# Virtana/accurate-aprilgroup-tracking

Measured on AMD Instinct MI355X. Metric: frames/sec (LK+PnP) on 1280x720 dodeca stream, higher is better.
Workload: dtype u8/i64 (LK), f64 (PnP); 1 GPU; c2: 1 x 1280x720 stream(s) per GPU, 12 tags/48 corners, 3-level LK 21x21, iterative PnP with motion-model guess; streams_per_gpu=1, frames_resident=HBM ring 368 slots (323 MiB), parallelism=stream-per-GPU x1, RCCL all_gather of poses once per block

## Files before the change

### accurate_aprilgroup_tracking_amd/csrc/agt_device.h

```cpp
#pragma once
#include <hip/hip_runtime.h>
#include <stdint.h>
#include <float.h>

#define AGT_WAVE 64

__device__ __forceinline__ int agt_reflect101(int p, int len)
{
    if ((unsigned)p < (unsigned)len) return p;
    if (len == 1) return 0;
    do {
        p = p < 0 ? -p : 2 * (len - 1) - p;
    } while ((unsigned)p >= (unsigned)len);
    return p;
}

template <int CTRL>
__device__ __forceinline__ int agt_dpp_i32(int v)
{
    return __builtin_amdgcn_update_dpp(0, v, CTRL, 0xf, 0xf, true);
}

__device__ __forceinline__ long long agt_dpp_add_i64_step(long long v, int lo, int hi)
{
// ... 26 lines not shown
}

__device__ __forceinline__ int agt_uniform(int v) { return __builtin_amdgcn_readfirstlane(v); }
__device__ __forceinline__ float agt_uniform(float v)
{
    return __int_as_float(__builtin_amdgcn_readfirstlane(__float_as_int(v)));
}

#pragma clang fp contract(fast)

__device__ __forceinline__ double agt_rcp(double x)
{
    double r = __builtin_amdgcn_rcp(x);
    double e = __builtin_fma(-x, r, 1.0);
    r = __builtin_fma(r, e, r);
    e = __builtin_fma(-x, r, 1.0);
    return __builtin_fma(r, e, r);
}
__device__ __forceinline__ double agt_rcp1(double x)
{
    const double r = __builtin_amdgcn_rcp(x);
    return __builtin_fma(r, __builtin_fma(-x, r, 1.0), r);
}
__device__ __forceinline__ double agt_sqrtp(double x)
{
    if (x == 0.0) return 0.0;
    const double y = __builtin_amdgcn_rsq(x);
    double g = x * y, h = 0.5 * y;
    double r = __builtin_fma(-h, g, 0.5);
    g = __builtin_fma(g, r, g); h = __builtin_fma(h, r, h);
    const double d = __builtin_fma(-g, g, x);
    return __builtin_fma(d, h, g);
}


__device__ __forceinline__ void agt_sincos(double x, double& s, double& c)
{
    if (!(x < 1048576.0)) { sincos(x, &s, &c); return; }
    const double k = rint(x * 6.36619772367581382433e-01);
    double r = fma(-k, 1.57079632673412561417e+00, x);
    r = fma(-k, 6.07710050650619224932e-11, r);
    const double z = r * r;
    const double sp = fma(z, fma(z, fma(z, fma(z, fma(z, 1.58969099521155010221e-10, -2.50507602534068634195e-08), 2.75573137070700676789e-06),
                                       -1.98412698298579493134e-04), 8.33333333332248946124e-03), -1.66666666666666324348e-01);
    const double cp = fma(z, fma(z, fma(z, fma(z, fma(z, -1.13596475577881948265e-11, 2.08757232129817482790e-09), -2.75573143513906633035e-07),
                                       2.48015872894767294178e-05), -1.38888888888741095749e-03), 4.16666666666666019037e-02);
    const double sr = fma(r * z, sp, r);
    const double cr = fma(z * z, cp, fma(z, -0.5, 1.0));
    const int q = (int)k & 3;
    const double ss = (q & 1) ? cr : sr, cc = (q & 1) ? sr : cr;
    s = (q & 2) ? -ss : ss;
    c = ((q + 1) & 2) ? -cc : cc;
}

template <bool JAC>
__device__ __forceinline__ void agt_rodrigues(const double r_in[3], double R[9], double G[9])
{
    double rx = r_in[0], ry = r_in[1], rz = r_in[2];
    const double t2 = rx * rx + ry * ry + rz * rz;
    const double theta = agt_sqrtp(t2);
    const bool tiny = theta < DBL_EPSILON;
    double s, c;
    agt_sincos(theta, s, c);
    const double c1 = 1.0 - c, itheta = agt_rcp(tiny ? 1.0 : theta);
    if (JAC) {
        double a, bq;
        if (theta < 1e-2) {
            a = 0.5 - t2 * (1.0 / 24.0 - t2 * (1.0 / 720.0 - t2 * (1.0 / 40320.0)));
            bq = 1.0 / 6.0 - t2 * (1.0 / 120.0 - t2 * (1.0 / 5040.0 - t2 * (1.0 / 362880.0)));
        } else {
            const double it2 = itheta * itheta;
            a = c1 * it2;
            bq = (theta - s) * it2 * itheta;
        }
        const double d = 1.0 - bq * t2;
        const double g[9] = { d + bq * rx * rx, bq * rx * ry - a * rz, bq * rx * rz + a * ry,
                              bq * rx * ry + a * rz, d + bq * ry * ry, bq * ry * rz - a * rx,
                              bq * rx * rz - a * ry, bq * ry * rz + a * rx, d + bq * rz * rz };
#pragma unroll
        for (int i = 0; i < 9; i++) G[i] = tiny ? ((i % 4 == 0) ? 1.0 : 0.0) : g[i];
    }
    rx *= itheta; ry *= itheta; rz *= itheta;
    const double rrt[9] = { rx * rx, rx * ry, rx * rz, rx * ry, ry * ry, ry * rz, rx * rz, ry * rz, rz * rz };
    const double r_x[9] = { 0, -rz, ry, rz, 0, -rx, -ry, rx, 0 };
#pragma unroll
    for (int k = 0; k < 9; k++) {
        const double v = c * ((k % 4 == 0) ? 1.0 : 0.0) + c1 * rrt[k] + s * r_x[k];
        R[k] = tiny ? ((k % 4 == 0) ? 1.0 : 0.0) : v;
    }
}

struct AgtCamera {
    double fx, fy, cx, cy;
    double k[12];
    const double* tilt;
};

__device__ __forceinline__ void agt_tilt_apply(const double* M, double x, double y, double& xo, double& yo, double* d)
{
    double v[3];
#pragma unroll
    for (int r = 0; r < 3; r++) { double a = 0.0; a += M[r * 3] * x; a += M[r * 3 + 1] * y; a += M[r * 3 + 2] * 1.0; v[r] = a; }
    const double ip = v[2] != 0.0 ? 1.0 / v[2] : 1.0;
    xo = ip * v[0]; yo = ip * v[1];
    if (d) {
        const double ip2 = ip * ip;
#pragma unroll
        for (int r = 0; r < 2; r++)
#pragma unroll
            for (int c = 0; c < 2; c++) d[r * 2 + c] = (M[r * 3 + c] * v[2] - M[6 + c] * v[r]) * ip2;
    }
}

template <bool JAC, bool DIST = true>
__device__ __forceinline__ void agt_project(const AgtCamera& cam, const double R[9], const double G[9],
                                            const double t[3], double X, double Y, double Z,
                                            double& u, double& v, double jr[6], double jt[6])
{
    const double* k = cam.k;
    const double wx = R[0] * X + R[1] * Y + R[2] * Z;
    const double wy = R[3] * X + R[4] * Y + R[5] * Z;
    const double wz = R[6] * X + R[7] * Y + R[8] * Z;
    double x = wx + t[0];
    double y = wy + t[1];
    double z = wz + t[2];
    z = z != 0.0 ? agt_rcp(z) : 1.0;
    x *= z; y *= z;
    if (!DIST) {
        u = x * cam.fx + cam.cx;
        v = y * cam.fy + cam.cy;
        if (JAC) {
            jt[0] = cam.fx * z; jt[1] = 0.0; jt[2] = cam.fx * (-x * z);
            jt[3] = 0.0; jt[4] = cam.fy * z; jt[5] = cam.fy * (-y * z);
#pragma unroll
            for (int j = 0; j < 3; j++) {
                const double gx = G[j], gy = G[3 + j], gz = G[6 + j];
                const double dx0 = gy * wz - gz * wy;
                const double dy0 = gz * wx - gx * wz;
                const double dz0 = gx * wy - gy * wx;
                jr[j] = cam.fx * (z * (dx0 - x * dz0));
                jr[3 + j] = cam.fy * (z * (dy0 - y * dz0));
            }
// ... 227 lines not shown
```

### accurate_aprilgroup_tracking_amd/csrc/agt_lk_chain_body.h

```cpp
#pragma once
#include "agt_lk_body.h"

#ifdef AGT_STEP_STAMPS
__device__ unsigned long long agt_chain_stamps[4 * 16];
__device__ unsigned agt_chain_counts[8];
#define CCOUNT(i, n) do { if (threadIdx.x == 0) atomicAdd(&agt_chain_counts[i], (unsigned)(n)); } while (0)
#define CSTAMP(i) do { if (pidx == 0 && threadIdx.x == 0 && k < 4) agt_chain_stamps[k * 16 + (i)] = __builtin_amdgcn_s_memtime(); } while (0)
extern "C" int agt_debug_chain_stamps(unsigned long long* host64)
{
    return (int)hipMemcpyFromSymbol(host64, HIP_SYMBOL(agt_chain_stamps), sizeof(agt_chain_stamps));
}
extern "C" int agt_debug_chain_counts(unsigned* host8)
{
    return (int)hipMemcpyFromSymbol(host8, HIP_SYMBOL(agt_chain_counts), sizeof(agt_chain_counts));
}
#else
#define CSTAMP(i)
#define CCOUNT(i, n)
#endif

#ifdef AGT_CHAIN_REPS
__device__ int agt_chain_reps[8] = { 1, 1, 1, 1, 1, 1, 1, 1 };
extern "C" int agt_debug_chain_reps(const int* host8) { return (int)hipMemcpyToSymbol(HIP_SYMBOL(agt_chain_reps), host8, 32); }
#define CREPS(i) for (int rep_ = 0, n_ = *(volatile int*)&agt_chain_reps[i]; rep_ < n_; rep_++)
// ... 276 lines not shown
            }
            if (sv) *reinterpret_cast<int2*>(sDall + l * (K::SD / 4) + sY * DW + sX) = make_int2(val[0], val[1]);
        }
        lds_barrier();
        CSTAMP(3);

        int Iv[NLEV][C::NPX], Ix[NLEV][C::NPX], Iy[NLEV][C::NPX];
        CREPS(1)
#pragma unroll
        for (int l = 0; l < NLEV; l++) {
            int iw00, iw01, iw10, iw11;
            bilinear_weights(fa[l], fb[l], iw00, iw01, iw10, iw11);
            const uint8_t* s0 = lds + offS[l];
            const int* sD = sDall + l * (K::SD / 4);
            int a0 = 0, a1 = 0, a2 = 0;
#pragma unroll
            for (int q = 0; q < C::NPX; q++) {
                const uint8_t* p = s0 + oW[q];
                const int iv = descale(bil4(p[0], p[1], p[JP], p[JP + 1], iw00, iw01, iw10, iw11), W_BITS - 5);
                const int* d = sD + oD[q];
                const int d00 = d[0], d01 = d[1], d10 = d[DW], d11 = d[DW + 1];
                const int ix = descale(bil4((short)d00, (short)d01, (short)d10, (short)d11, iw00, iw01, iw10, iw11), W_BITS);
                const int iy = descale(bil4(d00 >> 16, d01 >> 16, d10 >> 16, d11 >> 16, iw00, iw01, iw10, iw11), W_BITS);
                Iv[l][q] = pv[q] ? iv : 0; Ix[l][q] = pv[q] ? ix : 0; Iy[l][q] = pv[q] ? iy : 0;
                a0 += __mul24(Ix[l][q], Ix[l][q]); a1 += __mul24(Ix[l][q], Iy[l][q]); a2 += __mul24(Iy[l][q], Iy[l][q]);
            }
            red[(3 * l) * T + tid] = a0; red[(3 * l + 1) * T + tid] = a1; red[(3 * l + 2) * T + tid] = a2;
        }
        lds_barrier();
        CREPS(2)
        for (int l = wave; l < NLEV; l += NW) {
            int s4[3];
#pragma unroll
            for (int i = 0; i < 3; i++) {
                const int* r = red + (3 * l + i) * T + lane;
                s4[i] = r[0] + r[64] + r[128] + r[192];
            }
            int lo[3], hi[3];
            wave_sum2_i32(s4[0] & 0xffff, s4[1] & 0xffff, lo[0], lo[1]);
            wave_sum2_i32(s4[2] & 0xffff, s4[0] >> 16, lo[2], hi[0]);
            wave_sum2_i32(s4[1] >> 16, s4[2] >> 16, hi[1], hi[2]);
            float A[3];
#pragma unroll
            for (int i = 0; i < 3; i++) A[i] = fmaf((float)hi[i], 65536.f, (float)lo[i]) * FLT_SCALE;
            const float D = A[0] * A[2] - A[1] * A[1];
            const float minEig = (A[2] + A[0] - sqrtf((A[0] - A[2]) * (A[0] - A[2]) + 4.f * A[1] * A[1])) / (float)(2 * WIN * WIN);
            const bool ok = ((lvA >> l) & 1) && !((double)minEig < min_eig_threshold || D < FLT_EPSILON);
            if (lane == 0) {
                float* o = lvl + l * 8;
                o[0] = A[0]; o[1] = A[1]; o[2] = A[2]; o[3] = ok ? 1.f / D : 0.f; o[4] = ok ? 1.f : 0.f;
            }
        }
        lds_barrier();
        if (owed && tid == 0) lk_arrive(owed, b);
        owed = nullptr;
        CSTAMP(4);

        int st = 1;
        float outx = 0.f, outy = 0.f;
        bool pre = false;
        uint32_t tn[NLEV][C::JLD];
        int nox[NLEV], noy[NLEV], nmask = 0;
#pragma unroll
        for (int l = 0; l < NLEV; l++) { nox[l] = noy[l] = 0; }
#pragma unroll
        for (int level = NLEV - 1; level >= 0; level--) {
            if (level > maxl) continue;
            const float scale = lk_level_scale(level);
            float nextx, nexty;
            if (level == maxl) { nextx = px * scale; nexty = py * scale; }
            else { nextx = outx * 2.f; nexty = outy * 2.f; }
            outx = nextx; outy = nexty;
            CSTAMP(8 + level * 2);
            if (level == 0 && k + 1 < nf) {
                const LkFrameIo<NLEV> nio = frame(k + 1);
                if (agt_uniform((int)(all_safe && !nio.bad))) {
                    CREPS(4) {
                    nmask = 0;
#pragma unroll
                    for (int l = 0; l < NLEV; l++) {
                        typedef const __attribute__((address_space(1))) uint8_t* G8;
                        typedef const __attribute__((address_space(1))) uint32_t* G32;
                        const float sc = lk_level_scale(l);
                        const int cx = agt_uniform((int)floorf(outx * sc - halfw)), cy = agt_uniform((int)floorf(outy * sc - halfw));
                        const int w = gw[l], h = gh[l];
                        const long pitch = gpitch[l], bstride = gbs[l];
                        const int ox = cx - MARGIN, oy = cy - MARGIN, ax0 = ox & ~3;
                        const bool ok = l <= maxl && ax0 >= 0 && ax0 + 4 * C::JNDW <= w && oy >= 0 && oy + JT <= h;
                        const int lx = ok ? ax0 : 0, ly = ok ? oy : 0;
                        const uint8_t* img = l <= maxl ? nio.imgJ[l] : nio.imgJ[0];
                        const G8 base = (G8)img + (long)b * (l <= maxl ? bstride : 0) + (long)ly * (l <= maxl ? pitch : 0) + lx;
#pragma unroll
                        for (int q = 0; q < C::JLD; q++) tn[l][q] = *(G32)(base + toff[l][q]);
                        nox[l] = ox; noy[l] = oy;
                        nmask |= ok ? 1 << l : 0;
                    }
                    }
                    pre = true;
                }
            }
            if (!((lvA >> level) & 1)) { if (level == 0) st = 0; continue; }
            const float4 lv4 = *reinterpret_cast<const float4*>(lvl + level * 8);
            if (!agt_uniform((int)(lvl[level * 8 + 4] != 0.f))) { if (level == 0) st = 0; continue; }
            AgtLevel LJ;
            LJ.ptr = nullptr; LJ.w = gw[level]; LJ.h = gh[level]; LJ.pitch = gpitch[level]; LJ.bstride = gbs[level];
            const uint8_t* imgJ = io.imgJ[level] + (long)b * LJ.bstride;
            uint8_t* sJ = lds + (cur * NLEV + level) * K::TILE;
            const float a11 = agt_uniform(lv4.x), a12 = agt_uniform(lv4.y), a22 = agt_uniform(lv4.z), D = agt_uniform(lv4.w);
            int iv[C::NPX], ix[C::NPX], iy[C::NPX];
#pragma unroll
            for (int q = 0; q < C::NPX; q++) { iv[q] = Iv[level][q]; ix[q] = Ix[level][q]; iy[q] = Iy[level][q]; }
            int jx0 = jox[level], jy0 = joy[level];

            nextx -= halfw; nexty -= halfw;
            float pdx = 0.f, pdy = 0.f;
            int iw00, iw01, iw10, iw11;
            float bx0, bx1, by0, by1;
            auto set_box = [&]() {
                const int lx = jx0 > -WIN ? jx0 : -WIN, hx = (jx0 + JT - WIN - 1 < LJ.w - 1 ? jx0 + JT - WIN - 1 : LJ.w - 1) + 1;
                const int ly = jy0 > -WIN ? jy0 : -WIN, hy = (jy0 + JT - WIN - 1 < LJ.h - 1 ? jy0 + JT - WIN - 1 : LJ.h - 1) + 1;
                bx0 = (float)lx; bx1 = (float)hx; by0 = (float)ly; by1 = (float)hy;
            };
            set_box();
            int slow = agt_uniform((int)!(nextx >= bx0 && nextx < bx1 && nexty >= by0 && nexty < by1));
            for (int j = 0; j < max_count; j++) {
                const float fx = floorf(nextx), fy = floorf(nexty);
                if (slow) {
                    const int inx = agt_uniform((int)fx), iny = agt_uniform((int)fy);
                    if (inx < -WIN || inx >= LJ.w || iny < -WIN || iny >= LJ.h) {
                        if (level == 0) st = 0;
                        break;
                    }
                    if (inx < jx0 || inx + WIN >= jx0 + JT || iny < jy0 || iny + WIN >= jy0 + JT) {
                        jx0 = inx - MARGIN; jy0 = iny - MARGIN;
                        uint32_t t[C::JLD];
                        block_sync<NW>();
                        tile_load<JT, C::JNDW, T, C::JLD, true>(imgJ, LJ.w, LJ.h, LJ.pitch, jx0, jy0, tid, t);
                        tile_store<JT, C::JNDW, T>(sJ, tid, t);
                        __builtin_amdgcn_s_waitcnt(0x0F70);
                        block_sync<NW>();
                        set_box();
                    }
                }
                const int inx = (int)fx, iny = (int)fy;
                const uint8_t* q0 = sJ + __mul24(iny - jy0, JP) + (inx - jx0) + (jx0 - (jx0 & ~3));
                int tap[C::NPX][4];
#pragma unroll
                for (int q = 0; q < C::NPX; q++) {
                    const uint8_t* c = q0 + oW[q];
                    tap[q][0] = c[0]; tap[q][1] = c[1]; tap[q][2] = c[JP]; tap[q][3] = c[JP + 1];
                }
                __builtin_amdgcn_sched_barrier(0);
                bilinear_weights(nextx - fx, nexty - fy, iw00, iw01, iw10, iw11);
                int bsum[2] = { 0, 0 };
#pragma unroll
                for (int q = 0; q < C::NPX; q++) {
// ... 63 lines not shown
```

### accurate_aprilgroup_tracking_amd/csrc/agt_pnp_body.h

```cpp
#pragma once
#include <type_traits>
#include <cstddef>
#include "agt_device.h"
#include "agt_kernels.h"

#ifdef AGT_PNP_STAMPS
__device__ unsigned long long agt_pnp_stamps[64];
#define PSTAMP(i) do { if (b == 0 && threadIdx.x == 0) agt_pnp_stamps[i] = __builtin_amdgcn_s_memtime(); } while (0)
#define PSTAMPM(i) do { int mk_; asm volatile("s_mov_b32 %0, %1" : "=s"(mk_) : "n"(0xbeef00 + (i))); PSTAMP(i); } while (0)
extern "C" int agt_debug_pnp_stamps(unsigned long long* host64)
{
    return (int)hipMemcpyFromSymbol(host64, HIP_SYMBOL(agt_pnp_stamps), sizeof(agt_pnp_stamps));
}
#else
#define PSTAMP(i)
#define PSTAMPM(i)
#endif

#pragma clang fp contract(fast)

namespace agt_pnp {

constexpr int NACC = 28;
constexpr int SLAB = 65;
constexpr int MAX_PPL = 4;

__device__ __forceinline__ void pnp_sync()
{
    __builtin_amdgcn_fence(__ATOMIC_RELEASE, "wavefront");
    __builtin_amdgcn_wave_barrier();
    __builtin_amdgcn_fence(__ATOMIC_ACQUIRE, "wavefront");
}

struct PnpShared {
    double part[NACC * SLAB];
    double tot[NACC + 4];
    double LL[144];
    double vec[48];
    unsigned long long tab[5 * AGT_MAX_GROUP];
    int seq;
    int late;
    int coop[2];
    AgtTrackState ts;
};

typedef __attribute__((address_space(3))) AgtTrackState AgtTrackStateLds;

template <int K, bool READBACK = true>
__device__ __forceinline__ void wave_reduce_slab(double (&vals)[K], PnpShared& sh, int lane)
{
    static_assert(K <= NACC, "the slab holds NACC rows");
    pnp_sync();
#pragma unroll
    for (int k = 0; k < K; k++) sh.part[k * SLAB + lane] = vals[k];
    pnp_sync();
    const int k = lane & 31, h = lane >> 5;
    double s = 0.0;
    if (k < K) {
        const double* p = &sh.part[k * SLAB + 32 * h];
#pragma unroll 8
        for (int i = 0; i < 32; i++) s += p[i];
    }
    s += __shfl_xor(s, 32);
    if (lane < K) sh.tot[lane] = s;
    pnp_sync();
    if (READBACK) {
#pragma unroll
        for (int i = 0; i < K; i++) vals[i] = sh.tot[i];
    }
}

__device__ __forceinline__ double dswap32(double a, double b, double& b_out)
{
    const auto lo = __builtin_amdgcn_permlane32_swap((unsigned)__double2loint(a), (unsigned)__double2loint(b), false, false);
    const auto hi = __builtin_amdgcn_permlane32_swap((unsigned)__double2hiint(a), (unsigned)__double2hiint(b), false, false);
    b_out = __hiloint2double((int)hi[1], (int)lo[1]);
    return __hiloint2double((int)hi[0], (int)lo[0]);
}
__device__ __forceinline__ double dswap16(double a, double b, double& b_out)
{
    const auto lo = __builtin_amdgcn_permlane16_swap((unsigned)__double2loint(a), (unsigned)__double2loint(b), false, false);
    const auto hi = __builtin_amdgcn_permlane16_swap((unsigned)__double2hiint(a), (unsigned)__double2hiint(b), false, false);
    b_out = __hiloint2double((int)hi[1], (int)lo[1]);
    return __hiloint2double((int)hi[0], (int)lo[0]);
}
template <int CTRL>
__device__ __forceinline__ double ddpp(double v)
{
    return __hiloint2double(agt_dpp_i32<CTRL>(__double2hiint(v)), agt_dpp_i32<CTRL>(__double2loint(v)));
// ... 179 lines not shown
        d = sqrt(d);
        const double djj = lane_bcast(d, j);
        const double id = 1.0 / djj;
        l[j] = (i == j) ? djj : s * id;
    }
    pnp_sync();
    if (lane < N) {
#pragma unroll
        for (int k = 0; k < N; k++) A[i * N + k] = l[k];
    }
    pnp_sync();
#pragma unroll
    for (int k = 0; k < N; k++) lt[k] = A[k * N + i];
    double dii = 0.0;
#pragma unroll
    for (int k = 0; k < N; k++) dii = (i == k) ? l[k] : dii;
    const double idii = 1.0 / dii;
    double x = 1.0 / sqrt((double)N) * ((i & 1) ? 0.9 : 1.1);
    for (int it = 0; it < 12; it++) {
        double acc = x, y = 0.0;
#pragma unroll
        for (int k = 0; k < N; k++) {
            const double yk = lane_bcast(acc * idii, k);
            y = (i == k) ? yk : y;
            acc -= l[k] * yk;
        }
        acc = y;
#pragma unroll
        for (int k = N - 1; k >= 0; k--) {
            const double xk = lane_bcast(acc * idii, k);
            x = (i == k) ? xk : x;
            acc -= lt[k] * xk;
        }
        const double nn = wave_sum_f64(lane < N ? x * x : 0.0);
        x *= 1.0 / sqrt(nn);
    }
    if (lane < N) v_out[lane] = x;
    pnp_sync();
}

__device__ inline void mat3_tmul(const double A[9], const double B[9], double C[9])
{
#pragma unroll
    for (int i = 0; i < 3; i++)
#pragma unroll
        for (int j = 0; j < 3; j++) C[i * 3 + j] = A[i] * B[j] + A[3 + i] * B[3 + j] + A[6 + i] * B[6 + j];
}
__device__ inline void mat3_tvec(const double A[9], const double v[3], double o[3])
{
#pragma unroll
    for (int i = 0; i < 3; i++) o[i] = A[i] * v[0] + A[3 + i] * v[1] + A[6 + i] * v[2];
}

template <typename TS>
__device__ inline int motion_model_update(TS* ts, int lane, const double curr[6], bool curr_t_f32,
                                          const double prev[6], bool prev_t_f32, const double Rc[9], const double* st)
{
    double Rp[9];
#pragma unroll
    for (int i = 0; i < 9; i++) Rp[i] = st[24 + i];
    double d[3], tran_vel[3], rot_vel[9];
#pragma unroll
    for (int i = 0; i < 3; i++)
        d[i] = (curr_t_f32 && prev_t_f32) ? (double)((float)prev[3 + i] - (float)curr[3 + i]) : prev[3 + i] - curr[3 + i];
    mat3_tvec(Rc, d, tran_vel);
    mat3_tmul(Rc, Rp, rot_vel);
    bool any_zero = false;
#pragma unroll
    for (int i = 0; i < 9; i++) any_zero |= rot_vel[i] == 0.0;
#pragma unroll
    for (int i = 0; i < 3; i++) any_zero |= tran_vel[i] == 0.0;
    if (any_zero) return AGT_TRK_ZERO_VELOCITY;
    const int n_before = ts->n_vel;
    double old_rv[9], old_tv[3];
    const int old_slot = n_before >= 2 ? 1 : 0;
#pragma unroll
    for (int i = 0; i < 9; i++) old_rv[i] = st[old_slot * 9 + i];
#pragma unroll
    for (int i = 0; i < 3; i++) old_tv[i] = st[18 + old_slot * 3 + i];
    const int n_after = n_before >= 2 ? 2 : n_before + 1;
    if (lane == 0) {
        if (n_before >= 2) {
            for (int i = 0; i < 9; i++) ts->rot_vel[0][i] = old_rv[i];
            for (int i = 0; i < 3; i++) ts->tran_vel[0][i] = old_tv[i];
        }
        const int slot = n_after - 1;
        for (int i = 0; i < 9; i++) ts->rot_vel[slot][i] = rot_vel[i];
        for (int i = 0; i < 3; i++) ts->tran_vel[slot][i] = tran_vel[i];
        ts->n_vel = n_after;
    }
    if (n_after < 2) return 0;
    double dv[3], tran_acc[3], rot_acc[9];
#pragma unroll
    for (int i = 0; i < 3; i++) dv[i] = old_tv[i] - tran_vel[i];
    mat3_tvec(rot_vel, dv, tran_acc);
    mat3_tmul(rot_vel, old_rv, rot_acc);
    const double sy = agt_sqrtp(rot_acc[0] * rot_acc[0] + rot_acc[3] * rot_acc[3]);
    const bool sing = sy < 1e-6;
    double ay, ax;
    if (lane == 0) { ay = sing ? -rot_acc[5] : rot_acc[7]; ax = sing ? rot_acc[4] : rot_acc[8]; }
    else if (lane == 1) { ay = -rot_acc[6]; ax = sy; }
    else { ay = sing ? 0.0 : rot_acc[3]; ax = sing ? 1.0 : rot_acc[0]; }
    double sn, cs;
    {
        const double r = agt_sqrtp(ax * ax + ay * ay);
        if (r > 0.0) {
            const double ir = agt_rcp(r), c = ax * ir, sv = ay * ir;
            if (c >= 0.0) { cs = agt_sqrtp(0.5 * (1.0 + c)); sn = sv * agt_rcp(2.0 * cs); }
            else { const double a = agt_sqrtp(0.5 * (1.0 - c)); sn = copysign(a, ay); cs = fabs(sv) * agt_rcp(2.0 * a); }
        } else { cs = 1.0; sn = 0.0; }
    }
    const double sx = lane_bcast(sn, 0), cx = lane_bcast(cs, 0);
    const double sy2 = lane_bcast(sn, 1), cy = lane_bcast(cs, 1);
    const double sz = lane_bcast(sn, 2), cz = lane_bcast(cs, 2);
    const double Rx[9] = { 1, 0, 0, 0, cx, -sx, 0, sx, cx };
    const double Ry[9] = { cy, 0, sy2, 0, 1, 0, -sy2, 0, cy };
    const double Rz[9] = { cz, -sz, 0, sz, cz, 0, 0, 0, 1 };
    double Tm[9], RA[9], M[9], Rpred[9], tp[3], tpred[3];
    agt_mat3_mul(Ry, Rx, Tm);
    agt_mat3_mul(Rz, Tm, RA);
    agt_mat3_mul(RA, rot_vel, M);
    agt_mat3_mul(M, Rp, Rpred);
#pragma unroll
    for (int i = 0; i < 3; i++) tp[i] = prev[3 + i];
#pragma unroll
    for (int i = 0; i < 3; i++)
        tpred[i] = (M[i * 3] * tp[0] + M[i * 3 + 1] * tp[1] + M[i * 3 + 2] * tp[2]) +
                   (RA[i * 3] * tran_vel[0] + RA[i * 3 + 1] * tran_vel[1] + RA[i * 3 + 2] * tran_vel[2] + 0.5 * tran_acc[i]);
    double rpred[3];
    agt_rodrigues_inv(Rpred, rpred);
    if (lane == 0) {
        for (int i = 0; i < 3; i++) { ts->guess[i] = rpred[i]; ts->guess[3 + i] = (double)(float)tpred[i]; }
        ts->guess_t_f32 = 1;
    }
    return 0;
}

struct PnpNoHook { __device__ __forceinline__ void operator()() const {} };

template <typename T, int PPL, typename Hook = PnpNoHook, bool LDS_STATE = false, int COOP = 1, bool OPAQUE = false>
__device__ __forceinline__ void pnp_body(const AgtPnpParams& P, int b, PnpShared& sh, const void* img_p, const uint8_t* mask_p,
                                         double* so_p, int extra_flags = 0, Hook before_state = Hook())
{
    using TS = typename std::conditional<LDS_STATE, AgtTrackStateLds, AgtTrackState>::type;
    static_assert(COOP == 1 || (PPL == 1 && COOP * 32 * 3 <= NACC * SLAB), "cooperating waves hold one point per lane; slabs live in sh.part");
    int tid_ = (int)threadIdx.x;
    if constexpr (OPAQUE) asm volatile("" : "+v"(tid_));
    const int lane = tid_ & (AGT_WAVE - 1);
    const int wave = COOP > 1 ? agt_uniform(tid_ >> 6) : 0;
    const bool master = wave == 0;
    const bool writer = lane == 0 && master;
    const int n = P.n;
    int slab_sel = 0;
    double* const tot = COOP > 1 ? &sh.part[2 * COOP * 32 + wave * 32] : sh.tot;
    auto coop_sum = [&](double v) -> double {
        if constexpr (COOP == 1) return v;
        else {
            double* slot = &sh.part[slab_sel * COOP * 32];
            if (lane == 0) slot[wave * 32] = v;
            __syncthreads();
            double s_ = slot[0];
#pragma unroll
            for (int w = 1; w < COOP; w++) s_ += slot[w * 32];
            slab_sel ^= 1;
            return s_;
        }
    };
    PSTAMP(0);
    AgtCamera cam;
    load_cam<T>(P.cam, cam);

    double X[PPL], Y[PPL], Z[PPL], mu_[PPL], mv_[PPL];
    bool use[PPL];
    const T* obj = reinterpret_cast<const T*>(P.obj) + (long)b * P.obj_bstride;
    const T* img = reinterpret_cast<const T*>(img_p) + (long)b * n * 2;
    const uint8_t* mask = mask_p ? mask_p + (long)b * n : nullptr;
    int cnt = 0;
#pragma unroll
    for (int q = 0; q < PPL; q++) {
        const int i = lane + (q * COOP + wave) * AGT_WAVE;
        use[q] = i < n && (!mask || mask[i] != 0);
        X[q] = Y[q] = Z[q] = mu_[q] = mv_[q] = 0.0;
        if (use[q]) {
            X[q] = (double)obj[i * 3]; Y[q] = (double)obj[i * 3 + 1]; Z[q] = (double)obj[i * 3 + 2];
            mu_[q] = (double)img[i * 2]; mv_[q] = (double)img[i * 2 + 1];
            cnt++;
        }
    }
    if (P.seed_pts) {
        for (int i = lane + wave * AGT_WAVE; i < n; i += AGT_WAVE * COOP) {
            P.seed_pts[((long)b * n + i) * 2] = (float)img[i * 2]; P.seed_pts[((long)b * n + i) * 2 + 1] = (float)img[i * 2 + 1];
            P.seed_status[(long)b * n + i] = (!mask || mask[i] != 0) ? 1 : 0;
        }
    }
    if (P.tag_gate) {
        cnt = 0;
#pragma unroll
        for (int q = 0; q < PPL; q++) {
            int u = use[q] ? 1 : 0;
            u &= agt_dpp_i32<0xB1>(u);
            u &= agt_dpp_i32<0x4E>(u);
            use[q] = u != 0;
            if (!use[q]) X[q] = Y[q] = Z[q] = mu_[q] = mv_[q] = 0.0;
            cnt += u;
        }
    }
    const int n_used = (int)coop_sum((double)agt_wave_sum_i64(cnt));
// ... 378 lines not shown
                    const int u = ui[a][c];
                    sh.LL[a * 12 + c] = s0[u];           sh.LL[a * 12 + 4 + c] = 0.0;          sh.LL[a * 12 + 8 + c] = sx[u];
                    sh.LL[(4 + a) * 12 + c] = 0.0;       sh.LL[(4 + a) * 12 + 4 + c] = s0[u];  sh.LL[(4 + a) * 12 + 8 + c] = sy[u];
                    sh.LL[(8 + a) * 12 + c] = sx[u];     sh.LL[(8 + a) * 12 + 4 + c] = sy[u];  sh.LL[(8 + a) * 12 + 8 + c] = sq[u];
                }
        }
        pnp_sync();
        smallest_eigvec_wave<12>(sh.LL, sh.vec, lane);
        if (lane == 0) {
            double* v = sh.vec;
            double RR[9] = { v[0], v[1], v[2], v[4], v[5], v[6], v[8], v[9], v[10] };
            double tt[3] = { v[3], v[7], v[11] };
            if (agt_det3(RR) < 0) {
                for (int i = 0; i < 9; i++) RR[i] = -RR[i];
                for (int i = 0; i < 3; i++) tt[i] = -tt[i];
            }
            double sc = 0;
            for (int i = 0; i < 9; i++) sc += RR[i] * RR[i];
            sc = sqrt(sc);
            double Wr[3], U[9], Vt[9], Rm[9];
            agt_svd3(RR, Wr, U, Vt);
            agt_mat3_mul(U, Vt, Rm);
            double nr = 0;
            for (int i = 0; i < 9; i++) nr += Rm[i] * Rm[i];
            nr = sqrt(nr);
            double rv[3];
            agt_rodrigues_inv(Rm, rv);
            sh.vec[32] = rv[0]; sh.vec[33] = rv[1]; sh.vec[34] = rv[2];
            sh.vec[35] = tt[0] * nr / sc; sh.vec[36] = tt[1] * nr / sc; sh.vec[37] = tt[2] * nr / sc;
        }
        pnp_sync();
#pragma unroll
        for (int i = 0; i < 6; i++) param[i] = sh.vec[32 + i];
        }
    }

    double JtJ[21], JtErr[6];
    double prevParam[6];
    double prevErrNorm = DBL_MAX, errNorm = 0.0;
    int lambdaLg10 = -3, iters = 0;
    double lambda = 1e-3;
    const int max_iter = 20;
    const double epsilon = (double)FLT_EPSILON;

    bool has_dist = false;
#pragma unroll
    for (int i = 0; i < 12; i++) has_dist |= cam.k[i] != 0.0;
    has_dist |= cam.tilt != nullptr;
    double rex[PPL], rey[PPL];
#pragma unroll
    for (int q = 0; q < PPL; q++) { rex[q] = 0.0; rey[q] = 0.0; }

    double Rlast[9];
    auto evaluate_t = [&](int mode, auto DIST) -> double {
        constexpr bool D = decltype(DIST)::value;
        const bool needJ = mode != 0;
        double R[9], G[9];
        if (mode == 2) PSTAMPM(48);
        if (needJ) agt_rodrigues<true>(param, R, G); else agt_rodrigues<false>(param, R, G);
#pragma unroll
        for (int i = 0; i < 9; i++) Rlast[i] = R[i];
        if (mode == 2) PSTAMPM(49);
        if (needJ) {
            double acc[NACC];
#pragma unroll
            for (int i = 0; i < NACC; i++) acc[i] = 0.0;
#pragma unroll
            for (int q = 0; q < PPL; q++) if (PPL > 1 || use[q]) {
                double u, v, jr[6], jt[6];
                agt_project<true, D>(cam, R, G, param + 3, X[q], Y[q], Z[q], u, v, jr, jt);
                const double m = (PPL > 1 && !use[q]) ? 0.0 : 1.0;
                const double ex = (u - mu_[q]) * m, ey = (v - mv_[q]) * m;
                rex[q] = ex; rey[q] = ey;
                const double Jx[6] = { jr[0] * m, jr[1] * m, jr[2] * m, jt[0] * m, jt[1] * m, jt[2] * m };
                const double Jy[6] = { jr[3] * m, jr[4] * m, jr[5] * m, jt[3] * m, jt[4] * m, jt[5] * m };
                int idx = 0;
#pragma unroll
                for (int a = 0; a < 6; a++) {
#pragma unroll
                    for (int c = a; c < 6; c++) acc[idx++] += Jx[a] * Jx[c] + Jy[a] * Jy[c];
                    acc[21 + a] += Jx[a] * ex + Jy[a] * ey;
                }
                acc[27] += ex * ex + ey * ey;
            }
            if (mode == 2) PSTAMPM(50);
            if constexpr (COOP == 1) wave_reduce_bfly<NACC>(acc, tot, lane);
            else {
                double* slot = &sh.part[slab_sel * COOP * 32];
                wave_reduce_bfly<NACC>(acc, slot + wave * 32, lane);
                __syncthreads();
                if (lane < NACC) {
                    double s_ = slot[lane];
#pragma unroll
                    for (int w = 1; w < COOP; w++) s_ += slot[w * 32 + lane];
                    tot[lane] = s_;
                }
                pnp_sync();
                slab_sel ^= 1;
            }
            if (mode == 2) {
                PSTAMPM(51);
                return tot[27];
            }
#pragma unroll
            for (int i = 0; i < 21; i++) JtJ[i] = tot[i];
#pragma unroll
            for (int i = 0; i < 6; i++) JtErr[i] = tot[21 + i];
            return tot[27];
        }
        double e2 = 0.0;
#pragma unroll
        for (int q = 0; q < PPL; q++) if (PPL > 1 || use[q]) {
            double u, v;
            agt_project<false, D>(cam, R, G, param + 3, X[q], Y[q], Z[q], u, v, nullptr, nullptr);
            const double m = (PPL > 1 && !use[q]) ? 0.0 : 1.0;
            const double ex = (u - mu_[q]) * m, ey = (v - mv_[q]) * m;
            rex[q] = ex; rey[q] = ey;
            e2 += ex * ex + ey * ey;
        }
        return coop_sum(wave_sum_f64(e2));
    };
    auto evaluate = [&](int mode) -> double {
        return has_dist ? evaluate_t(mode, std::true_type{}) : evaluate_t(mode, std::false_type{});
    };
    auto commit_candidate = [&]() {
#pragma unroll
        for (int i = 0; i < 21; i++) JtJ[i] = tot[i];
#pragma unroll
        for (int i = 0; i < 6; i++) JtErr[i] = tot[21 + i];
    };
    auto residuals_same_rotation = [&](auto DIST) {
        constexpr bool D = decltype(DIST)::value;
#pragma unroll
        for (int q = 0; q < PPL; q++) if (use[q]) {
            double u, v;
            agt_project<false, D>(cam, Rlast, nullptr, param + 3, X[q], Y[q], Z[q], u, v, nullptr, nullptr);
            rex[q] = u - mu_[q]; rey[q] = v - mv_[q];
        }
    };

    auto step = [&]() {
        double A[36], dx[6];
        int idx = 0;
#pragma unroll
        for (int a = 0; a < 6; a++)
#pragma unroll
            for (int c = a; c < 6; c++) { A[a * 6 + c] = JtJ[idx]; A[c * 6 + a] = JtJ[idx]; idx++; }
#pragma unroll
        for (int a = 0; a < 6; a++) A[a * 7] *= 1.0 + lambda;
        if (!agt_solve6(A, JtErr, dx)) {
            flags |= AGT_PNP_SINGULAR;
#pragma unroll
            for (int a = 0; a < 6; a++) dx[a] = 0.0;
        }
#pragma unroll
        for (int a = 0; a < 6; a++) param[a] = prevParam[a] - dx[a];
    };

    PSTAMP(1);
    double e2 = evaluate(1);
    PSTAMP(2);
    for (;;) {
#pragma unroll
        for (int i = 0; i < 6; i++) prevParam[i] = param[i];
        if (iters == 0) prevErrNorm = sqrt(e2);
        double rel = 0.0, e2cand = 0.0;
        bool last = false;
        for (;;) {
            PSTAMP(8 + iters * 4 + 0);
            step();
            PSTAMP(8 + iters * 4 + 1);
            double dn = 0.0, pn = 0.0;
#pragma unroll
            for (int i = 0; i < 6; i++) { const double d = param[i] - prevParam[i]; dn += d * d; pn += prevParam[i] * prevParam[i]; }
            rel = sqrt(dn) / (sqrt(pn) + DBL_EPSILON);
            last = iters + 1 >= max_iter || rel < epsilon;
            e2cand = evaluate(last ? 0 : 2);
            errNorm = sqrt(e2cand);
            PSTAMP(8 + iters * 4 + 2);
            if (errNorm > prevErrNorm) { ++lambdaLg10; lambda *= 10.0; if (lambdaLg10 <= 16) continue; }
            break;
        }
        if (lambdaLg10 - 1 >= -16) { lambdaLg10 -= 1; lambda *= 0.1; } else { lambdaLg10 = -16; lambda = 1e-16; }
        ++iters;
        if (last) break;
        prevErrNorm = errNorm;
        commit_candidate();
        e2 = e2cand;
        PSTAMP(8 + (iters - 1) * 4 + 3);
    }
    PSTAMP(3);

    const bool tvec_f32 = ts && use_guess && guess_f32;
    if (tvec_f32) {
#pragma unroll
        for (int i = 3; i < 6; i++) param[i] = (double)(float)param[i];
    }

    double esum = 0.0;
    {
        if (tvec_f32) { if (has_dist) residuals_same_rotation(std::true_type{}); else residuals_same_rotation(std::false_type{}); }
#pragma unroll
        for (int q = 0; q < PPL; q++) if (use[q]) esum += sqrt(rex[q] * rex[q] + rey[q] * rey[q]);
        esum = coop_sum(wave_sum_f64(esum)) / n_used;
    }
    PSTAMP(4);
    if (!master) return;
    if (ts) {
        const bool accepted = esum < P.gate_px;
        int tflags = flags;
        if (writer && use_guess) {
            for (int i = 0; i < 6; i++) ts->guess[i] = param[i];
        }
        if (accepted && had_guess && P.enhance_ape)
            tflags |= motion_model_update(ts, lane, param, tvec_f32, unchanged_prev, prev_f32 != 0, Rlast, sh.vec);
        if (writer) {
            if (accepted) {
                if (!had_guess || !P.enhance_ape) {
                    for (int i = 0; i < 6; i++) ts->guess[i] = param[i];
                    ts->guess_t_f32 = 0; ts->has_guess = 1;
                }
                if (!(tflags & AGT_TRK_ZERO_VELOCITY)) {
                    for (int i = 0; i < 6; i++) ts->prev[i] = param[i];
                    for (int i = 0; i < 9; i++) ts->prev_R[i] = Rlast[i];
                    ts->prev_t_f32 = tvec_f32 ? 1 : 0; ts->has_prev = 1;
                }
            } else {
                ts->has_guess = 0;
            }
            ts->frame++;
            PSTAMP(5);
            if (P.dense_pose) {
                double* rc = P.dense_rec + (long)b * AGT_DENSE_STRIDE;
                for (int i = 0; i < 6; i++) { P.dense_pose[(long)b * 6 + i] = param[i]; rc[i] = param[i]; }
                for (int i = 6; i < AGT_DENSE_STRIDE; i++) rc[i] = 0.0;
                P.dense_done[b] = accepted ? 0 : 1;
            }
            if (so_p) {
                double* so = so_p + (long)b * AGT_STATE_STRIDE;
                for (int i = 0; i < 6; i++) so[i] = param[i];
                so[AGT_ST_OK] = accepted ? 1.0 : 0.0; so[AGT_ST_ERR] = esum; so[AGT_ST_NTRACK] = n_used;
                so[AGT_ST_ITERS] = iters; so[AGT_ST_GUESS] = use_guess ? 1.0 : 0.0; so[AGT_ST_FLAGS] = tflags;
                so[AGT_ST_TVEC_F32] = tvec_f32 ? 1.0 : 0.0;
                for (int i = AGT_ST_TVEC_F32 + 1; i < AGT_STATE_STRIDE; i++) so[i] = 0.0;
            }
        }
        if (accepted && P.reproject && P.corners_rw) {
            double R[9], G[9];
            agt_rodrigues<false>(param, R, G);
            float* cw = P.corners_rw + (long)b * n * 2;
            for (int i = lane; i < n; i += AGT_WAVE) {
                double u, v;
                agt_project<false>(cam, R, G, param + 3, (double)obj[i * 3], (double)obj[i * 3 + 1], (double)obj[i * 3 + 2],
                                   u, v, nullptr, nullptr);
                cw[i * 2] = (float)u; cw[i * 2 + 1] = (float)v;
                if (P.status_rw) P.status_rw[(long)b * n + i] = 1;
            }
        }
        return;
    }
    if (writer) {
#pragma unroll
        for (int i = 0; i < 6; i++) P.pose[(long)b * 6 + i] = param[i];
        if (P.info) {
            P.info[b * 4 + AGT_INFO_OK] = 1; P.info[b * 4 + AGT_INFO_ITERS] = iters;
            P.info[b * 4 + AGT_INFO_NUSED] = n_used; P.info[b * 4 + AGT_INFO_FLAGS] = flags;
        }
        if (P.err) P.err[b] = esum;
// ... 7 lines not shown
```

Baseline: 78160 frames/s.

## Overlap PnP motion model with final residuals and double-buffer LM accumulators

Splits Rodrigues into a head (sqrt/sincos) and a tail so the head is computed before the convergence check. It double-buffers the reduced JtJ/JtErr totals so an accepted candidate only flips an index instead of copying. The motion model is split into branch-free head, tail and store stages and runs speculatively next to the final residual sum when one point sits per lane. LK level validity for all levels is loaded once after the barrier instead of per level. This shortens serial dependency chains in the single-wave PnP tail, in exchange for more registers and LDS and motion-model work that is discarded when the pose is rejected.

```diff
diff --git a/accurate_aprilgroup_tracking_amd/csrc/agt_device.h b/accurate_aprilgroup_tracking_amd/csrc/agt_device.h
--- a/accurate_aprilgroup_tracking_amd/csrc/agt_device.h
+++ b/accurate_aprilgroup_tracking_amd/csrc/agt_device.h
@@ -102,17 +102,36 @@
     s = (q & 2) ? -ss : ss;
     c = ((q + 1) & 2) ? -cc : cc;
 }
-
+__device__ __forceinline__ double agt_sqrtp_sel(double x)
+{
+    const bool z = x == 0.0;
+    const double xs = z ? 1.0 : x;
+    const double y = __builtin_amdgcn_rsq(xs);
+    double g = xs * y, h = 0.5 * y;
+    double r = __builtin_fma(-h, g, 0.5);
+    g = __builtin_fma(g, r, g); h = __builtin_fma(h, r, h);
+    const double d = __builtin_fma(-g, g, xs);
+    return z ? 0.0 : __builtin_fma(d, h, g);
+}
+
+struct AgtRodHead { double t2, theta, s, c, c1, itheta; bool tiny; };
+__device__ __forceinline__ AgtRodHead agt_rodrigues_head(const double r_in[3])
+{
+    AgtRodHead h;
+    const double rx = r_in[0], ry = r_in[1], rz = r_in[2];
+    h.t2 = rx * rx + ry * ry + rz * rz;
+    h.theta = agt_sqrtp(h.t2);
+    h.tiny = h.theta < DBL_EPSILON;
+    agt_sincos(h.theta, h.s, h.c);
+    h.c1 = 1.0 - h.c; h.itheta = agt_rcp(h.tiny ? 1.0 : h.theta);
+    return h;
+}
 template <bool JAC>
-__device__ __forceinline__ void agt_rodrigues(const double r_in[3], double R[9], double G[9])
+__device__ __forceinline__ void agt_rodrigues_tail(const double r_in[3], const AgtRodHead& h, double R[9], double G[9])
 {
     double rx = r_in[0], ry = r_in[1], rz = r_in[2];
-    const double t2 = rx * rx + ry * ry + rz * rz;
-    const double theta = agt_sqrtp(t2);
-    const bool tiny = theta < DBL_EPSILON;
-    double s, c;
-    agt_sincos(theta, s, c);
-    const double c1 = 1.0 - c, itheta = agt_rcp(tiny ? 1.0 : theta);
+    const double t2 = h.t2, theta = h.theta, s = h.s, c = h.c, c1 = h.c1, itheta = h.itheta;
+    const bool tiny = h.tiny;
     if (JAC) {
         double a, bq;
         if (theta < 1e-2) {
@@ -138,6 +157,11 @@
         const double v = c * ((k % 4 == 0) ? 1.0 : 0.0) + c1 * rrt[k] + s * r_x[k];
         R[k] = tiny ? ((k % 4 == 0) ? 1.0 : 0.0) : v;
     }
+}
+template <bool JAC>
+__device__ __forceinline__ void agt_rodrigues(const double r_in[3], double R[9], double G[9])
+{
+    agt_rodrigues_tail<JAC>(r_in, agt_rodrigues_head(r_in), R, G);
 }
 
 struct AgtCamera {
diff --git a/accurate_aprilgroup_tracking_amd/csrc/agt_lk_chain_body.h b/accurate_aprilgroup_tracking_amd/csrc/agt_lk_chain_body.h
--- a/accurate_aprilgroup_tracking_amd/csrc/agt_lk_chain_body.h
+++ b/accurate_aprilgroup_tracking_amd/csrc/agt_lk_chain_body.h
@@ -352,6 +352,18 @@
             }
         }
         lds_barrier();
+        constexpr bool LVL_AT_ONCE = NLEV <= 3;
+        float4 lvc[LVL_AT_ONCE ? NLEV : 1];
+        int lvU = lvA;
+        if constexpr (LVL_AT_ONCE) {
+            int um = 0;
+#pragma unroll
+            for (int l = 0; l < NLEV; l++) {
+                lvc[l] = *reinterpret_cast<const float4*>(lvl + l * 8);
+                um |= (lvl[l * 8 + 4] != 0.f) ? 1 << l : 0;
+            }
+            lvU = agt_uniform(um) & lvA;
+        }
         if (owed && tid == 0) lk_arrive(owed, b);
         owed = nullptr;
         CSTAMP(4);
@@ -399,9 +411,13 @@
                     pre = true;
                 }
             }
-            if (!((lvA >> level) & 1)) { if (level == 0) st = 0; continue; }
-            const float4 lv4 = *reinterpret_cast<const float4*>(lvl + level * 8);
-            if (!agt_uniform((int)(lvl[level * 8 + 4] != 0.f))) { if (level == 0) st = 0; continue; }
+            if (!((lvU >> level) & 1)) { if (level == 0) st = 0; continue; }
+            float4 lv4;
+            if constexpr (LVL_AT_ONCE) lv4 = lvc[level];
+            else {
+                lv4 = *reinterpret_cast<const float4*>(lvl + level * 8);
+                if (!agt_uniform((int)(lvl[level * 8 + 4] != 0.f))) { if (level == 0) st = 0; continue; }
+            }
             AgtLevel LJ;
             LJ.ptr = nullptr; LJ.w = gw[level]; LJ.h = gh[level]; LJ.pitch = gpitch[level]; LJ.bstride = gbs[level];
             const uint8_t* imgJ = io.imgJ[level] + (long)b * LJ.bstride;
diff --git a/accurate_aprilgroup_tracking_amd/csrc/agt_pnp_body.h b/accurate_aprilgroup_tracking_amd/csrc/agt_pnp_body.h
--- a/accurate_aprilgroup_tracking_amd/csrc/agt_pnp_body.h
+++ b/accurate_aprilgroup_tracking_amd/csrc/agt_pnp_body.h
@@ -34,7 +34,7 @@
 
 struct PnpShared {
     double part[NACC * SLAB];
-    double tot[NACC + 4];
+    double tot[2 * (NACC + 4)];
     double LL[144];
     double vec[48];
     unsigned long long tab[5 * AGT_MAX_GROUP];
@@ -320,63 +320,62 @@
     for (int i = 0; i < 3; i++) o[i] = A[i] * v[0] + A[3 + i] * v[1] + A[6 + i] * v[2];
 }
 
+struct MotionOut {
+    bool zero_vel;
+    bool predict;
+    int n_before, n_after;
+    double rot_vel[9], tran_vel[3], old_rv[9], old_tv[3];
+    double Rpred[9], rpred[3], tpred[3];
+};
 template <typename TS>
-__device__ inline int motion_model_update(TS* ts, int lane, const double curr[6], bool curr_t_f32,
-                                          const double prev[6], bool prev_t_f32, const double Rc[9], const double* st)
+__device__ __forceinline__ void motion_model_head(const TS* ts, int lane, const double curr[6], bool curr_t_f32,
+                                                  const double prev[6], bool prev_t_f32, const double Rc[9], const double* st, MotionOut& o)
 {
     double Rp[9];
 #pragma unroll
     for (int i = 0; i < 9; i++) Rp[i] = st[24 + i];
-    double d[3], tran_vel[3], rot_vel[9];
+    double d[3];
 #pragma unroll
     for (int i = 0; i < 3; i++)
         d[i] = (curr_t_f32 && prev_t_f32) ? (double)((float)prev[3 + i] - (float)curr[3 + i]) : prev[3 + i] - curr[3 + i];
-    mat3_tvec(Rc, d, tran_vel);
-    mat3_tmul(Rc, Rp, rot_vel);
+    mat3_tvec(Rc, d, o.tran_vel);
+    mat3_tmul(Rc, Rp, o.rot_vel);
     bool any_zero = false;
 #pragma unroll
-    for (int i = 0; i < 9; i++) any_zero |= rot_vel[i] == 0.0;
-#pragma unroll
-    for (int i = 0; i < 3; i++) any_zero |= tran_vel[i] == 0.0;
-    if (any_zero) return AGT_TRK_ZERO_VELOCITY;
+    for (int i = 0; i < 9; i++) any_zero |= o.rot_vel[i] == 0.0;
+#pragma unroll
+    for (int i = 0; i < 3; i++) any_zero |= o.tran_vel[i] == 0.0;
+    o.zero_vel = any_zero;
     const int n_before = ts->n_vel;
-    double old_rv[9], old_tv[3];
     const int old_slot = n_before >= 2 ? 1 : 0;
 #pragma unroll
-    for (int i = 0; i < 9; i++) old_rv[i] = st[old_slot * 9 + i];
-#pragma unroll
-    for (int i = 0; i < 3; i++) old_tv[i] = st[18 + old_slot * 3 + i];
-    const int n_after = n_before >= 2 ? 2 : n_before + 1;
-    if (lane == 0) {
-        if (n_before >= 2) {
-            for (int i = 0; i < 9; i++) ts->rot_vel[0][i] = old_rv[i];
-            for (int i = 0; i < 3; i++) ts->tran_vel[0][i] = old_tv[i];
-        }
-        const int slot = n_after - 1;
-        for (int i = 0; i < 9; i++) ts->rot_vel[slot][i] = rot_vel[i];
-        for (int i = 0; i < 3; i++) ts->tran_vel[slot][i] = tran_vel[i];
-        ts->n_vel = n_after;
-    }
-    if (n_after < 2) return 0;
+    for (int i = 0; i < 9; i++) o.old_rv[i] = st[old_slot * 9 + i];
+#pragma unroll
+    for (int i = 0; i < 3; i++) o.old_tv[i] = st[18 + old_slot * 3 + i];
+    o.n_before = n_before;
+    o.n_after = n_before >= 2 ? 2 : n_before + 1;
+    o.predict = !any_zero && o.n_after >= 2;
     double dv[3], tran_acc[3], rot_acc[9];
 #pragma unroll
-    for (int i = 0; i < 3; i++) dv[i] = old_tv[i] - tran_vel[i];
-    mat3_tvec(rot_vel, dv, tran_acc);
-    mat3_tmul(rot_vel, old_rv, rot_acc);
-    const double sy = agt_sqrtp(rot_acc[0] * rot_acc[0] + rot_acc[3] * rot_acc[3]);
+    for (int i = 0; i < 3; i++) dv[i] = o.old_tv[i] - o.tran_vel[i];
+    mat3_tvec(o.rot_vel, dv, tran_acc);
+    mat3_tmul(o.rot_vel, o.old_rv, rot_acc);
+    const double sy = agt_sqrtp_sel(rot_acc[0] * rot_acc[0] + rot_acc[3] * rot_acc[3]);
     const bool sing = sy < 1e-6;
-    double ay, ax;
-    if (lane == 0) { ay = sing ? -rot_acc[5] : rot_acc[7]; ax = sing ? rot_acc[4] : rot_acc[8]; }
-    else if (lane == 1) { ay = -rot_acc[6]; ax = sy; }
-    else { ay = sing ? 0.0 : rot_acc[3]; ax = sing ? 1.0 : rot_acc[0]; }
+    const double ay0 = sing ? -rot_acc[5] : rot_acc[7], ax0 = sing ? rot_acc[4] : rot_acc[8];
+    const double ay2 = sing ? 0.0 : rot_acc[3], ax2 = sing ? 1.0 : rot_acc[0];
+    const double ay = lane == 0 ? ay0 : (lane == 1 ? -rot_acc[6] : ay2);
+    const double ax = lane == 0 ? ax0 : (lane == 1 ? sy : ax2);
     double sn, cs;
     {
-        const double r = agt_sqrtp(ax * ax + ay * ay);
-        if (r > 0.0) {
-            const double ir = agt_rcp(r), c = ax * ir, sv = ay * ir;
-            if (c >= 0.0) { cs = agt_sqrtp(0.5 * (1.0 + c)); sn = sv * agt_rcp(2.0 * cs); }
-            else { const double a = agt_sqrtp(0.5 * (1.0 - c)); sn = copysign(a, ay); cs = fabs(sv) * agt_rcp(2.0 * a); }
-        } else { cs = 1.0; sn = 0.0; }
+        const double r = agt_sqrtp_sel(ax * ax + ay * ay);
+        const bool rpos = r > 0.0;
+        const double ir = agt_rcp(rpos ? r : 1.0), c = ax * ir, sv = ay * ir;
+        const double a = agt_sqrtp_sel(0.5 * (1.0 + __builtin_fabs(c)));
+        const double h = agt_rcp(2.0 * a);
+        const bool cpos = c >= 0.0;
+        const double sn1 = cpos ? sv * h : copysign(a, ay), cs1 = cpos ? a : __builtin_fabs(sv) * h;
+        cs = rpos ? cs1 : 1.0; sn = rpos ? sn1 : 0.0;
     }
     const double sx = lane_bcast(sn, 0), cx = lane_bcast(cs, 0);
     const double sy2 = lane_bcast(sn, 1), cy = lane_bcast(cs, 1);
@@ -384,21 +383,40 @@
     const double Rx[9] = { 1, 0, 0, 0, cx, -sx, 0, sx, cx };
     const double Ry[9] = { cy, 0, sy2, 0, 1, 0, -sy2, 0, cy };
     const double Rz[9] = { cz, -sz, 0, sz, cz, 0, 0, 0, 1 };
-    double Tm[9], RA[9], M[9], Rpred[9], tp[3], tpred[3];
+    double Tm[9], RA[9], M[9], tp[3];
     agt_mat3_mul(Ry, Rx, Tm);
     agt_mat3_mul(Rz, Tm, RA);
-    agt_mat3_mul(RA, rot_vel, M);
-    agt_mat3_mul(M, Rp, Rpred);
+    agt_mat3_mul(RA, o.rot_vel, M);
+    agt_mat3_mul(M, Rp, o.Rpred);
 #pragma unroll
     for (int i = 0; i < 3; i++) tp[i] = prev[3 + i];
 #pragma unroll
     for (int i = 0; i < 3; i++)
-        tpred[i] = (M[i * 3] * tp[0] + M[i * 3 + 1] * tp[1] + M[i * 3 + 2] * tp[2]) +
-                   (RA[i * 3] * tran_vel[0] + RA[i * 3 + 1] * tran_vel[1] + RA[i * 3 + 2] * tran_vel[2] + 0.5 * tran_acc[i]);
-    double rpred[3];
-    agt_rodrigues_inv(Rpred, rpred);
+        o.tpred[i] = (M[i * 3] * tp[0] + M[i * 3 + 1] * tp[1] + M[i * 3 + 2] * tp[2]) +
+                     (RA[i * 3] * o.tran_vel[0] + RA[i * 3 + 1] * o.tran_vel[1] + RA[i * 3 + 2] * o.tran_vel[2] + 0.5 * tran_acc[i]);
+}
+__device__ __forceinline__ void motion_model_tail(MotionOut& o)
+{
+    o.rpred[0] = o.rpred[1] = o.rpred[2] = 0.0;
+    if (o.predict) agt_rodrigues_inv(o.Rpred, o.rpred);
+}
+template <typename TS>
+__device__ __forceinline__ int motion_model_store(TS* ts, int lane, const MotionOut& o)
+{
+    if (o.zero_vel) return AGT_TRK_ZERO_VELOCITY;
     if (lane == 0) {
-        for (int i = 0; i < 3; i++) { ts->guess[i] = rpred[i]; ts->guess[3 + i] = (double)(float)tpred[i]; }
+        if (o.n_before >= 2) {
+            for (int i = 0; i < 9; i++) ts->rot_vel[0][i] = o.old_rv[i];
+            for (int i = 0; i < 3; i++) ts->tran_vel[0][i] = o.old_tv[i];
+        }
+        const int slot = o.n_after - 1;
+        for (int i = 0; i < 9; i++) ts->rot_vel[slot][i] = o.rot_vel[i];
+        for (int i = 0; i < 3; i++) ts->tran_vel[slot][i] = o.tran_vel[i];
+        ts->n_vel = o.n_after;
+    }
+    if (o.n_after < 2) return 0;
+    if (lane == 0) {
+        for (int i = 0; i < 3; i++) { ts->guess[i] = o.rpred[i]; ts->guess[3 + i] = (double)(float)o.tpred[i]; }
         ts->guess_t_f32 = 1;
     }
     return 0;
@@ -411,7 +429,7 @@
                                          double* so_p, int extra_flags = 0, Hook before_state = Hook())
 {
     using TS = typename std::conditional<LDS_STATE, AgtTrackStateLds, AgtTrackState>::type;
-    static_assert(COOP == 1 || (PPL == 1 && COOP * 32 * 3 <= NACC * SLAB), "cooperating waves hold one point per lane; slabs live in sh.part");
+    static_assert(COOP == 1 || (PPL == 1 && COOP * 32 * 4 <= NACC * SLAB), "cooperating waves hold one point per lane; slabs live in sh.part");
     int tid_ = (int)threadIdx.x;
     if constexpr (OPAQUE) asm volatile("" : "+v"(tid_));
     const int lane = tid_ & (AGT_WAVE - 1);
@@ -421,6 +439,7 @@
     const int n = P.n;
     int slab_sel = 0;
     double* const tot = COOP > 1 ? &sh.part[2 * COOP * 32 + wave * 32] : sh.tot;
+    constexpr int TOT_ALT = COOP > 1 ? COOP * 32 : NACC + 4;
     auto coop_sum = [&](double v) -> double {
         if constexpr (COOP == 1) return v;
         else {
@@ -905,12 +924,13 @@
     for (int q = 0; q < PPL; q++) { rex[q] = 0.0; rey[q] = 0.0; }
 
     double Rlast[9];
-    auto evaluate_t = [&](int mode, auto DIST) -> double {
+    int acc_sel = 0;
+    auto evaluate_t = [&](int mode, const AgtRodHead& hd, auto DIST) -> double {
         constexpr bool D = decltype(DIST)::value;
         const bool needJ = mode != 0;
         double R[9], G[9];
         if (mode == 2) PSTAMPM(48);
-        if (needJ) agt_rodrigues<true>(param, R, G); else agt_rodrigues<false>(param, R, G);
+        if (needJ) agt_rodrigues_tail<true>(param, hd, R, G); else agt_rodrigues_tail<false>(param, hd, R, G);
 #pragma unroll
         for (int i = 0; i < 9; i++) Rlast[i] = R[i];
         if (mode == 2) PSTAMPM(49);
@@ -937,7 +957,8 @@
                 acc[27] += ex * ex + ey * ey;
             }
             if (mode == 2) PSTAMPM(50);
-            if constexpr (COOP == 1) wave_reduce_bfly<NACC>(acc, tot, lane);
+            double* const dst = tot + (mode == 2 ? acc_sel ^ 1 : acc_sel) * TOT_ALT;
+            if constexpr (COOP == 1) wave_reduce_bfly<NACC>(acc, dst, lane);
             else {
                 double* slot = &sh.part[slab_sel * COOP * 32];
                 wave_reduce_bfly<NACC>(acc, slot + wave * 32, lane);
@@ -946,20 +967,18 @@
                     double s_ = slot[lane];
 #pragma unroll
                     for (int w = 1; w < COOP; w++) s_ += slot[w * 32 + lane];
-                    tot[lane] = s_;
+                    dst[lane] = s_;
                 }
                 pnp_sync();
                 slab_sel ^= 1;
             }
-            if (mode == 2) {
-                PSTAMPM(51);
-                return tot[27];
-            }
-#pragma unroll
-            for (int i = 0; i < 21; i++) JtJ[i] = tot[i];
-#pragma unroll
-            for (int i = 0; i < 6; i++) JtErr[i] = tot[21 + i];
-            return tot[27];
+            if (mode == 2) PSTAMPM(51);
+            const double e2_ = dst[27];
+#pragma unroll
+            for (int i = 0; i < 21; i++) JtJ[i] = dst[i];
+#pragma unroll
+            for (int i = 0; i < 6; i++) JtErr[i] = dst[21 + i];
+            return e2_;
         }
         double e2 = 0.0;
 #pragma unroll
@@ -973,14 +992,15 @@
         }
         return coop_sum(wave_sum_f64(e2));
     };
-    auto evaluate = [&](int mode) -> double {
-        return has_dist ? evaluate_t(mode, std::true_type{}) : evaluate_t(mode, std::false_type{});
+    auto evaluate = [&](int mode, const AgtRodHead& hd) -> double {
+        return has_dist ? evaluate_t(mode, hd, std::true_type{}) : evaluate_t(mode, hd, std::false_type{});
     };
-    auto commit_candidate = [&]() {
-#pragma unroll
-        for (int i = 0; i < 21; i++) JtJ[i] = tot[i];
-#pragma unroll
-        for (int i = 0; i < 6; i++) JtErr[i] = tot[21 + i];
+    auto reload_accepted = [&]() {
+        const double* src = tot + acc_sel * TOT_ALT;
+#pragma unroll
+        for (int i = 0; i < 21; i++) JtJ[i] = src[i];
+#pragma unroll
+        for (int i = 0; i < 6; i++) JtErr[i] = src[21 + i];
     };
     auto residuals_same_rotation = [&](auto DIST) {
         constexpr bool D = decltype(DIST)::value;
@@ -1011,34 +1031,42 @@
     };
 
     PSTAMP(1);
-    double e2 = evaluate(1);
+    double e2 = evaluate(1, agt_rodrigues_head(param));
     PSTAMP(2);
     for (;;) {
 #pragma unroll
         for (int i = 0; i < 6; i++) prevParam[i] = param[i];
         if (iters == 0) prevErrNorm = sqrt(e2);
+        double pn = 0.0;
+#pragma unroll
+        for (int i = 0; i < 6; i++) pn += prevParam[i] * prevParam[i];
+        const double pnorm = sqrt(pn) + DBL_EPSILON;
         double rel = 0.0, e2cand = 0.0;
         bool last = false;
         for (;;) {
             PSTAMP(8 + iters * 4 + 0);
             step();
             PSTAMP(8 + iters * 4 + 1);
-            double dn = 0.0, pn = 0.0;
-#pragma unroll
-            for (int i = 0; i < 6; i++) { const double d = param[i] - prevParam[i]; dn += d * d; pn += prevParam[i] * prevParam[i]; }
-            rel = sqrt(dn) / (sqrt(pn) + DBL_EPSILON);
+            const AgtRodHead hd = agt_rodrigues_head(param);
+            double dn = 0.0;
+#pragma unroll
+            for (int i = 0; i < 6; i++) { const double d = param[i] - prevParam[i]; dn += d * d; }
+            rel = sqrt(dn) / pnorm;
             last = iters + 1 >= max_iter || rel < epsilon;
-            e2cand = evaluate(last ? 0 : 2);
+            e2cand = evaluate(last ? 0 : 2, hd);
             errNorm = sqrt(e2cand);
             PSTAMP(8 + iters * 4 + 2);
-            if (errNorm > prevErrNorm) { ++lambdaLg10; lambda *= 10.0; if (lambdaLg10 <= 16) continue; }
+            if (errNorm > prevErrNorm) {
+                ++lambdaLg10; lambda *= 10.0;
+                if (lambdaLg10 <= 16) { if (!last) reload_accepted(); continue; }
+            }
             break;
         }
         if (lambdaLg10 - 1 >= -16) { lambdaLg10 -= 1; lambda *= 0.1; } else { lambdaLg10 = -16; lambda = 1e-16; }
         ++iters;
         if (last) break;
         prevErrNorm = errNorm;
-        commit_candidate();
+        acc_sel ^= 1;
         e2 = e2cand;
         PSTAMP(8 + (iters - 1) * 4 + 3);
     }
@@ -1051,7 +1079,19 @@
     }
 
     double esum = 0.0;
-    {
+    const bool model = ts && had_guess && P.enhance_ape;
+    constexpr bool BESIDE = COOP == 1 && PPL == 1;
+    MotionOut mo;
+    if (BESIDE && model) {
+        motion_model_head(ts, lane, param, tvec_f32, unchanged_prev, prev_f32 != 0, Rlast, sh.vec, mo);
+        double u, v;
+        if (has_dist) agt_project<false, true>(cam, Rlast, nullptr, param + 3, X[0], Y[0], Z[0], u, v, nullptr, nullptr);
+        else agt_project<false, false>(cam, Rlast, nullptr, param + 3, X[0], Y[0], Z[0], u, v, nullptr, nullptr);
+        const double ex = tvec_f32 ? u - mu_[0] : rex[0], ey = tvec_f32 ? v - mv_[0] : rey[0];
+        const double en = sqrt(ex * ex + ey * ey);
+        esum = wave_sum_f64(use[0] ? en : 0.0) / n_used;
+        motion_model_tail(mo);
+    } else {
         if (tvec_f32) { if (has_dist) residuals_same_rotation(std::true_type{}); else residuals_same_rotation(std::false_type{}); }
 #pragma unroll
         for (int q = 0; q < PPL; q++) if (use[q]) esum += sqrt(rex[q] * rex[q] + rey[q] * rey[q]);
@@ -1065,8 +1105,13 @@
         if (writer && use_guess) {
             for (int i = 0; i < 6; i++) ts->guess[i] = param[i];
         }
-        if (accepted && had_guess && P.enhance_ape)
-            tflags |= motion_model_update(ts, lane, param, tvec_f32, unchanged_prev, prev_f32 != 0, Rlast, sh.vec);
+        if (accepted && model) {
+            if constexpr (!BESIDE) {
+                motion_model_head(ts, lane, param, tvec_f32, unchanged_prev, prev_f32 != 0, Rlast, sh.vec, mo);
+                motion_model_tail(mo);
+            }
+            tflags |= motion_model_store(ts, lane, mo);
+        }
         if (writer) {
             if (accepted) {
                 if (!had_guess || !P.enhance_ape) {
```

New measurement: 78650 frames/s, median of 6. About the same (+0.6%).
